# lightbulb128/troy-nova

Hardware: AMD Instinct MI355X
Metric: homomorphic mul+relinearize ops/sec (CKKS mul+relin+rescale), N=16384 (higher is better)
Workload: dtype u64; 1 GPU; CKKS N=16384, 6x50-bit coeff modulus (K=6, L=5): multiply + relinearize + rescale_to_next (BASELINE configs[2]); batch_per_gpu=1024, entry=troyn_ckks_multiply_relinearize_rescale, parallelism=batch-sharded x1, keys broadcast once (RCCL), ranks=1, slowest_rank=0

## Files before the change

### troy-nova_amd/csrc/ntt_kernels.hpp

```cpp
#pragma once
#include "dev_math.hpp"
#include "dev_math_f64.hpp"
#include <type_traits>

namespace troyn {

constexpr int KS_MAX_KEYS = 64;
struct KeyPtrs { const u64* p[KS_MAX_KEYS]; };

struct NttArgs {
    const u64* in;
    u64* out;
    const DevModulus* mods;
    const void* tw;
    long long in_bstride, in_pstride, in_cstride;
    long long out_bstride, out_pstride, out_cstride;
    unsigned pcount, ncomp;
    unsigned table_start, table_count, mode, decomp;
    unsigned reduce_input;
    unsigned stream_loads;
    unsigned load_mode, store_mode;
    unsigned aux_mod;
    unsigned skip_diag;
    unsigned flags;
// ... 258 lines not shown
        const unsigned x0 = (unsigned)x, x1 = (unsigned)(x >> 32), w0 = (unsigned)wq, w1 = (unsigned)(wq >> 32);
        const u64 qh = (u64)x1 * w1 + __umulhi(x1, w0) + __umulhi(x0, w1);
        return w * x + qh * neg_q;
    }
    static __device__ __forceinline__ u64 csub4(u64 v, const Mod& m) {
        const u64 t = v + m.neg_four_q;
        return (long long)t < 0 ? v : t;
    }
    static __device__ __forceinline__ elem mac_zero() { return 0; }
    static __device__ __forceinline__ elem mac_in(u64 canonical, const Mod&) { return canonical; }
    static __device__ __forceinline__ u64 mac_to_lds(elem x, const Mod& m) { return final_fwd(x, m); }
    static __device__ __forceinline__ void mac(elem& acc, elem v, u64 key, const Mod& m) {
        acc = add_mod(acc, barrett128(v * key, mul_hi(v, key), m.q, m.ratio_lo, m.ratio_hi), m.q);
    }
    static __device__ __forceinline__ void mac_fix(elem&, const Mod&) {}
    static __device__ __forceinline__ u64 mac_final(elem acc, const Mod& m) { return final_fwd(acc, m); }
    static constexpr bool HAS_MAC_SHOUP = true;
    static __device__ __forceinline__ void mac_shoup(elem& acc, elem v, u64 key, u64 kq, const Mod& m) {
        acc = csub4(acc + shoup_lazy3(v, key, kq, m.neg_q), m);
    }
    static __device__ __forceinline__ tw_t tw_from_mem(const tw_mem v, const Mod&) { return make_ulonglong2(v.x, v.y); }
    static __device__ __forceinline__ elem load_first(u64 raw, bool reduce, const Mod& m) { return reduce ? barrett64(raw, m.q, m.ratio_hi) : raw; }
    template <int LM> static __device__ __forceinline__ elem load_io(const NttIo& io, u64 raw, bool reduce, const Mod& m) {
        return load_first(ntt_io_load<LM>(io, raw), reduce, m);
    }
    template <int SM> static __device__ __forceinline__ u64 store_prep(elem x, const Mod& m) { return final_fwd(x, m); }
    template <int SM> static __device__ __forceinline__ u64 store_io(const NttIo& io, u64 word, u64 prod, u64 addend, u64 destv, const Mod&) {
        return ntt_io_store<SM>(io, word, prod, addend, destv);
    }
    static __device__ __forceinline__ elem load_mid(u64 raw, const Mod&) { return raw; }
    static __device__ __forceinline__ u64 store_mid(elem x, const Mod&) { return x; }
    static __device__ __forceinline__ elem from_lds(u64 raw) { return raw; }
    static __device__ __forceinline__ u64 to_lds(elem x, const Mod&) { return x; }
    static __device__ __forceinline__ elem mid_fix(elem x, const Mod&) { return x; }
    static __device__ __forceinline__ elem mid_sum(elem x, elem y, const Mod& m) { return csub4(x + y, m); }
    static __device__ __forceinline__ void fwd(elem& a, elem& b, const tw_t w, const Mod& m) {
        const u64 u = csub4(a, m);
        const u64 v = shoup_lazy3(b, w.x, w.y, m.neg_q);
        a = u + v;
        b = u + m.four_q - v;
    }
    static __device__ __forceinline__ void inv(elem& a, elem& b, const tw_t w, const Mod& m) {
        const u64 u = a, v = b;
        a = csub4(u + v, m);
        b = shoup_lazy3(u + m.four_q - v, w.x, w.y, m.neg_q);
    }
    static __device__ __forceinline__ u64 final_inv(elem v, const Mod& m) {
        return shoup_lazy(final_fwd(v, m), m.ninv_op, m.ninv_quo, m.q);
    }
    static __device__ __forceinline__ void inv_fold(elem&, elem&, const Mod&) {}
    static __device__ __forceinline__ elem held_t(elem x, bool, const Mod&) { return x; }
    static __device__ __forceinline__ elem keep(elem x, const Mod& m) { return final_fwd(x, m); }
    static __device__ __forceinline__ elem prod(elem x, elem y, const Mod& m) {
        u64 lo, hi;
        mul128(x, y, lo, hi);
        return barrett128(lo, hi, m.q, m.ratio_lo, m.ratio_hi);
    }
    static __device__ __forceinline__ elem sum(elem x, elem y, const Mod& m) { return add_mod(x, y, m.q); }
    static __device__ __forceinline__ elem inv_in(elem x, const Mod&) { return x; }
    static __device__ __forceinline__ elem prod_in(u64 x, u64 y, const Mod& m) { return prod(x, y, m); }
    static __device__ __forceinline__ elem from_canon(u64 x) { return x; }
    static __device__ __forceinline__ u64 t_residue(u64 raw, bool is_u64, bool aux_bigger, const Mod& m) {
        const u64 t = is_u64 ? raw : f64_to_u64(f64_bits_to_double(raw));
        return aux_bigger ? barrett64(t, m.q, m.ratio_hi) : t;
    }
    template <bool TW> static __device__ __forceinline__ elem tail_in(const NttIo& io, u64 raw_s, u64 raw_l, const Mod& m) {
        const u64 rs = sub_mod(t_residue(raw_s, io.ts_u64, io.aux_bigger, m), io.hm_u, m.q);
        const u64 fl = sub_mod(t_residue(raw_l, io.tl_u64, io.aux2_bigger, m), io.hm2_u, m.q);
        return add_mod(shoup_mul(rs, io.inv.x, io.inv.y, m.q), fl, m.q);
    }
    static __device__ __forceinline__ u64 tail_out(const NttIo& io, u64 prod_word, elem y, const Mod& m) {
        return shoup_mul(sub_mod(prod_word, final_fwd(y, m), m.q), io.inv2.x, io.inv2.y, m.q);
    }
    template <bool TW> static __device__ __forceinline__ u64 last_out(const NttIo& io, elem xr, bool, u64 raw_s, const Mod& m) {
        const u64 ys = final_inv(xr, m);
        const u64 rs = sub_mod(t_residue(raw_s, io.ts_u64, io.aux_bigger, m), io.hm_u, m.q);
        const u64 l = sub_mod(ys, shoup_mul(rs, io.inv.x, io.inv.y, m.q), m.q);
        return add_mod(l, m.q >> 1, m.q);
    }
};

struct ArithF64 {
    static constexpr bool HAS_MAC_SHOUP = false;
    using elem = double;
// ... 37 lines not shown
        }
    }
    template <int SM> static __device__ __forceinline__ u64 store_prep(elem x, const Mod& m) {
        if constexpr (SM == NTT_STORE_PLAIN) return final_fwd(x, m);
        else return f64_double_to_bits(f64_corr(x, m.m));
    }
    template <int SM> static __device__ __forceinline__ u64 store_io(const NttIo& io, u64 word, u64 prod, u64 addend, u64 destv, const Mod& m) {
        if constexpr (SM == NTT_STORE_PLAIN) return word;
        else {
            const double y = f64_bits_to_double(word);
            double d = f64_mulc(f64_from_u64(prod) - y, io.inv_d, io.inv_pd, m.m.p);
            if constexpr (SM == NTT_STORE_KS_FINISH) {
                if (io.add_inplace) d += f64_from_u64(destv);
                if (io.ext1) d += f64_from_u64(addend);
            }
            return f64_canon(d, m.m);
        }
    }
    static __device__ __forceinline__ elem prod_in(u64 x, u64 y, const Mod& m) {
        return f64_mulq(f64_from_u64(x), f64_from_u64(y), m.m.inv_p, m.m.p);
    }
    static __device__ __forceinline__ elem tensor_term(unsigned k, u64 a0, u64 a1, u64 b0, u64 b1, const Mod& m) {
        return k == 0 ? prod_in(a0, b0, m) : prod_in(a0, b1, m) + prod_in(a1, b0, m);
    }
    static __device__ __forceinline__ elem round_fix(u64 x, double aux_q, double aux_half, double hm, const Mod& m) {
        double t = f64_from_u64(x) + aux_half;
        t = (t >= aux_q) ? t - aux_q : t;
        return f64_corr(t - hm, m.m);
    }
    static __device__ __forceinline__ double round_half(double x_canon, const Mod& m) {
        const double t = x_canon + 0.5 * (m.m.p - 1.0);
        return t >= m.m.p ? t - m.m.p : t;
    }
    static __device__ __forceinline__ double held_t(elem x, bool scaled, const Mod& m) {
        const double c = f64_corr(scaled ? x : f64_mulc(x, m.ninv, m.ninv_p, m.m.p), m.m);
        return round_half(c < 0.0 ? c + m.m.p : c, m);
    }
    static __device__ __forceinline__ elem round_fix_t(u64 t_bits, double hm, const Mod& m) { return f64_corr(f64_bits_to_double(t_bits) - hm, m.m); }
    static __device__ __forceinline__ elem round_fix_tw(u64 raw, bool is_u64, double hm, const Mod& m) {
        double t;
        if (is_u64) {
            const double h = (double)(unsigned)(raw >> 30) * 1073741824.0;
            const double lo = (double)((unsigned)raw & 0x3fffffffu);
            t = __builtin_fma(-__builtin_rint(h * m.m.inv_p), m.m.p, h) + lo;
        } else t = f64_bits_to_double(raw);
        return f64_corr(t - hm, m.m);
    }
    static __device__ __forceinline__ elem from_canon(u64 x) { return f64_from_u64(x); }
    template <bool TW> static __device__ __forceinline__ elem tail_in(const NttIo& io, u64 raw_s, u64 raw_l, const Mod& m) {
        const elem rs = TW ? round_fix_tw(raw_s, io.ts_u64, io.hm_d, m) : round_fix_t(raw_s, io.hm_d, m);
        const elem fl = TW ? round_fix_tw(raw_l, io.tl_u64, io.hm2_d, m) : round_fix_t(raw_l, io.hm2_d, m);
        return scale_by(rs, io.inv_d, m) + fl;
    }
    static __device__ __forceinline__ u64 tail_out(const NttIo& io, u64 prod_word, elem y, const Mod& m) {
        return canon_small(scale_by(f64_corr(f64_from_u64(prod_word) - y, m.m), io.inv2_d, m), m);
    }
    template <bool TW> static __device__ __forceinline__ u64 last_out(const NttIo& io, elem xr, bool scaled, u64 raw_s, const Mod& m) {
        const elem ys = scaled ? xr : f64_mulc(xr, m.ninv, m.ninv_p, m.m.p);
        const elem rs = TW ? round_fix_tw(raw_s, io.ts_u64, io.hm_d, m) : round_fix_t(raw_s, io.hm_d, m);
        double lc = f64_corr(ys - scale_by(rs, io.inv_d, m), m.m);
        lc = lc < 0.0 ? lc + m.m.p : lc;
        return f64_double_to_bits(round_half(lc, m));
    }
    static __device__ __forceinline__ u64 canon_small(elem x, const Mod& m) { return f64_to_u64(x < 0.0 ? x + m.m.p : x); }
    static __device__ __forceinline__ elem scale_by(elem x, double inv_d, const Mod& m) { return f64_mulq(x, inv_d, m.m.inv_p, m.m.p); }
    static __device__ __forceinline__ elem load_mid(u64 raw, const Mod& m) { return f64_corr(f64_bits_to_double(raw), m.m); }
    static __device__ __forceinline__ u64 store_mid(elem x, const Mod&) { return f64_double_to_bits(x); }
    static __device__ __forceinline__ elem from_lds(u64 raw) { return f64_bits_to_double(raw); }
    static __device__ __forceinline__ u64 to_lds(elem x, const Mod& m) { return f64_double_to_bits(f64_corr(x, m.m)); }
    static __device__ __forceinline__ elem mid_fix(elem x, const Mod& m) { return f64_corr(x, m.m); }
    static __device__ __forceinline__ elem mid_sum(elem x, elem y, const Mod& m) { return f64_corr(x, m.m) + y; }
    static __device__ __forceinline__ void fwd(elem& a, elem& b, const tw_t w, const Mod& m) {
        const double r = f64_mulq(b, w.x, m.m.inv_p, m.m.p);
        const double u = a;
        a = u + r;
        b = u - r;
    }
    static __device__ __forceinline__ void inv(elem& a, elem& b, const tw_t w, const Mod& m) {
        const double u = a, v = b;
        a = u + v;
        b = f64_mulq(u - v, w.x, m.m.inv_p, m.m.p);
    }
    static __device__ __forceinline__ u64 final_fwd(elem v, const Mod& m) { return f64_canon(v, m.m); }
    static __device__ __forceinline__ u64 final_inv(elem v, const Mod& m) { return f64_canon(f64_mulc(v, m.ninv, m.ninv_p, m.m.p), m.m); }
    static __device__ __forceinline__ elem keep(elem x, const Mod& m) { return f64_corr(x, m.m); }
    static __device__ __forceinline__ elem prod(elem x, elem y, const Mod& m) { return f64_mulq(x, y, m.m.inv_p, m.m.p); }
    static __device__ __forceinline__ elem sum(elem x, elem y, const Mod&) { return x + y; }
    static __device__ __forceinline__ elem inv_in(elem x, const Mod& m) { return f64_corr(x, m.m); }
};

__host__ __device__ constexpr unsigned ntt_wave_bits(int S, int EB, int TB) {
    unsigned m = 0;
    for (int p = 6; p < TB - EB; ++p) m |= 1u << (p < S ? p : p + EB);
    return m;
}

__host__ __device__ constexpr bool ROUNDS_OK(int G, int EB) { return (G + EB - 1) / EB > 1; }

template <class A, int LOGN, int LO, int G, int TB, int EB, bool INV, bool FIRST, bool LAST, bool KSMAC, int IOM, int REGIO = 0, bool HALF = false, bool SHFL = false>
__device__ __forceinline__ void ntt_pass_body(const NttArgs& a, const KeyPtrs* keys, u64* lds, unsigned bid, unsigned t, typename A::elem* xio = nullptr) {
    constexpr int C = TB - G;
    static_assert(!HALF || (!KSMAC && REGIO == 0), "half-word LDS tiles: plain and fused transform kernels only");
    static_assert(REGIO == 0 || REGIO == 3 || REGIO == 4 || (!KSMAC && IOM == 0 && C == 0 && (G + EB - 1) / EB > 1 && (REGIO == 1 ? (!INV && LAST) : (INV && FIRST && (REGIO == 2 || !LAST)))), "register hand-over: last forward / first inverse pass on whole tiles");
    static_assert(REGIO < 3 || REGIO == 5 || (std::is_same<A, ArithF64>::value && !KSMAC && !HALF && C == 0 && LO == 0 && G == TB && TB == LOGN && (G + EB - 1) / EB > 1 &&
                                (REGIO == 3 ? (INV && (IOM == 0 || IOM == NTT_FUSED_LAST_LIMB)) : (REGIO == 4 && !INV && IOM == NTT_FUSED_TAIL_RESCALE))),
                  "held T rows: whole-limb FP64 transforms of the merged chain tail");
    constexpr int E = 1 << EB;
    constexpr unsigned N = 1u << LOGN;
    constexpr int TILE_BITS = LOGN - TB;
    constexpr int NLB = LOGN - LO - G - C;
    static_assert(G >= 1 && C >= 0 && NLB >= 0 && TB >= EB, "bad NTT pass shape");
    constexpr int ROUNDS = (G + EB - 1) / EB;
    static_assert(!KSMAC || (!INV && FIRST && LAST && C == 0 && LO == 0 && ROUNDS > 1), "KSMAC needs a whole-limb forward tile");
    using elem = typename A::elem;
    using tw_t = typename A::tw_t;

    unsigned tile, j, k, b;
    if constexpr (KSMAC) {
        tile = 0; j = 0;
        const unsigned R = a.xcd_groups;
        if (R > 1) {
            const unsigned per = 8u * R, phase = a.batch * R;
            const unsigned q = bid % phase, r = q % per;
            k = (bid / phase) * R + r / 8u;
            b = (q / per) * 8u + (r % 8u);
        } else {
            b = bid % a.batch; k = bid / a.batch;
        }
        if (a.ks_row_mask) k = nth_set_bit(a.ks_row_mask, k);
    } else {
        tile = bid & ((1u << TILE_BITS) - 1); bid >>= TILE_BITS;
        unsigned g;
        if (IOM != 0 && TILE_BITS == 0 && a.xcd_groups) {
            const unsigned per = 8u * a.ncomp, full = (a.xcd_groups / 8u) * per;
            if (bid < full) { const unsigned r = bid % per; j = r / 8u; g = (bid / per) * 8u + (r % 8u); }
            else { const unsigned r = bid - full; j = r % a.ncomp; g = (a.xcd_groups / 8u) * 8u + r / a.ncomp; }
        } else {
            j = bid % a.ncomp; g = bid / a.ncomp;
        }
        k = g % a.pcount;
        b = g / a.pcount;
    }
    const unsigned top = tile >> NLB;
    const unsigned lb = tile & ((1u << NLB) - 1);

    if (!KSMAC && a.skip_diag && k == j && k < a.decomp) return;
    const unsigned mi = KSMAC ? a.table_start + ((k == a.decomp) ? a.table_count - 1 : k) : ntt_table_index(a, k, j);
    const typename A::Mod md = A::make(a.mods[mi]);
    typedef typename A::tw_mem tw_mem;
    typedef const tw_mem __attribute__((address_space(4)))* ctw_ptr;
    unsigned long long tw_addr = (unsigned long long)(reinterpret_cast<const tw_mem*>(a.tw) + (size_t)mi * N);
    ctw_ptr twc = (ctw_ptr)tw_addr;
    auto tw_load = [&](unsigned idx) -> tw_t { const tw_mem v = twc[idx]; return A::tw_from_mem(v, md); };
    const u64* __restrict__ gin = a.in + (long long)b * a.in_bstride + (KSMAC ? 0ll : (long long)k * a.in_pstride + (long long)j * a.in_cstride);
    u64* __restrict__ gout = a.out + (long long)b * a.out_bstride + (KSMAC ? (long long)k * a.out_cstride : (long long)k * a.out_pstride + (long long)j * a.out_cstride);

    auto gindex = [&](unsigned loc) -> unsigned {
        return (top << (LOGN - LO)) | ((loc >> C) << (LOGN - LO - G)) | (lb << C) | (loc & ((1u << C) - 1));
    };
    auto gpart = [](unsigned loc) constexpr -> unsigned { return ((loc >> C) << (LOGN - LO - G)) | (loc & ((1u << C) - 1)); };
    constexpr int LM = (FIRST && !KSMAC && !INV) ? (IOM == 1 ? (int)NTT_LOAD_KS_ROUND : IOM == 2 ? (int)NTT_LOAD_RESCALE : IOM == NTT_IOM_CENTRALIZE ? (int)NTT_LOAD_CENTRALIZE : (int)NTT_LOAD_PLAIN) : (int)NTT_LOAD_PLAIN;
    constexpr int SM = (LAST && !KSMAC && !INV) ? (IOM == 1 ? (int)NTT_STORE_KS_FINISH : IOM == 2 ? (int)NTT_STORE_RESCALE : (int)NTT_STORE_PLAIN) : (int)NTT_STORE_PLAIN;
    constexpr bool FUSED = IOM >= 3 && IOM <= 7;
    constexpr bool F_MULPAIR = IOM == NTT_FUSED_MULPAIR && FIRST;
    constexpr bool F_LAST = IOM == NTT_FUSED_LAST_LIMB || IOM == NTT_FUSED_LAST_LIMB_W, F_TR = IOM == NTT_FUSED_TAIL_RESCALE || IOM == NTT_FUSED_TAIL_RESCALE_W;
    constexpr bool TW = IOM == NTT_FUSED_LAST_LIMB_W || IOM == NTT_FUSED_TAIL_RESCALE_W;
    constexpr bool F_LAST_LD = F_LAST && FIRST, F_LAST_ST = F_LAST && LAST;
    constexpr bool F_TR_LD = F_TR && FIRST, F_TR_ST = F_TR && LAST;
    constexpr bool F_KC_ST = INV && LAST && IOM == 1 && !KSMAC;
    static_assert(!FUSED || !KSMAC, "fused chain: transform kernels");
    static_assert(!TW || std::is_same<A, ArithF64>::value, "the _W variants exist for the FP64 policy (the integer forms read either kind of T row)");
    static_assert(!FUSED || (INV == (IOM == NTT_FUSED_MULPAIR || F_LAST)), "fused chain: transform direction");
    NttIo io;
    if constexpr (FUSED) { io.load_mode = NTT_LOAD_PLAIN; io.store_mode = NTT_STORE_PLAIN; ntt_io_fused(io, a, b, k, j, mi); }
    else if constexpr (LM != NTT_LOAD_PLAIN || SM != NTT_STORE_PLAIN) io = ntt_io_make(a, b, k, j, mi, gout);
    else if constexpr (F_KC_ST) { io = ntt_io_make(a, b, k, j, mi, gout); io.in2 = a.in2 + (long long)b * a.in2_bstride + (long long)k * a.in2_pstride; }
    else { io.load_mode = NTT_LOAD_PLAIN; io.store_mode = NTT_STORE_PLAIN; }
    const long long mul_off = FUSED ? (long long)(a.mul_limb0 + j) * N : 0ll;

    elem x[E];
    elem acc0[KSMAC ? E : 1], acc1[KSMAC ? E : 1];
    const u64* __restrict__ key0 = nullptr;
    const u64* __restrict__ kq0 = nullptr;
    if constexpr (KSMAC) {
        static_for<0, E>([&](auto Rc) { acc0[decltype(Rc)::value] = A::mac_zero(); acc1[decltype(Rc)::value] = A::mac_zero(); });
    }
    const u64* const gin0 = gin;
    auto one_digit = [&](unsigned it) {
    if constexpr (KSMAC) {
        asm volatile("" : "+v"(t));
        unsigned tw_lo = (unsigned)__builtin_amdgcn_readfirstlane((int)(unsigned)tw_addr);
        unsigned tw_hi = (unsigned)__builtin_amdgcn_readfirstlane((int)(unsigned)(tw_addr >> 32));
        asm volatile("" : "+s"(tw_lo), "+s"(tw_hi));
        twc = (ctw_ptr)(((unsigned long long)tw_hi << 32) | tw_lo);
        gin = gin0 + (long long)it * a.in_cstride;
        key0 = keys->p[it] + (size_t)(mi - a.table_start) * N;
        kq0 = a.key_quo ? a.key_quo + (long long)it * a.key_quo_jstride + (size_t)(mi - a.table_start) * N : nullptr;
        if (a.skip_diag && it == k) {
            const unsigned lane = t & 63u, wbase = (t >> 6) * (64u * E);
            const u64* dg = a.ext0 + (long long)b * a.ext0_bstride + (long long)k * a.ext0_cstride;
            static_for<0, E / 2>([&](auto mc) {
// ... 32 lines not shown
            sync();
            static_for<0, E>([&](auto ic) { lds32[wa(ic)] = (unsigned)(w[decltype(ic)::value] >> 32); });
            sync();
            static_for<0, E>([&](auto ic) { constexpr int i = decltype(ic)::value; w[i] = ((u64)lds32[ra(ic)] << 32) | (unsigned)w[i]; });
        }
    };
    auto nothing = [] {};
    auto wave_sync = [] { __builtin_amdgcn_wave_barrier(); };
    auto wg_sync = [] { __syncthreads(); };
    (void)wg_sync;
    static_for<0, ROUNDS>([&](auto rc) {
        constexpr int r = decltype(rc)::value;
        constexpr int BHI = INV ? ((C + (r + 1) * EB - 1 < TB - 1) ? C + (r + 1) * EB - 1 : TB - 1) : TB - 1 - r * EB;
        constexpr int BLO = INV ? C + r * EB : ((TB - (r + 1) * EB > C) ? TB - (r + 1) * EB : C);
        constexpr int S = INV ? ((BLO < TB - EB) ? BLO : TB - EB) : ((TB - (r + 1) * EB > 0) ? TB - (r + 1) * EB : 0);
        static_assert(S >= 0 && S + EB <= TB && BLO >= S && BHI < S + EB && BLO <= BHI, "bad round window");
        const unsigned tlow = t & ((1u << S) - 1);
        const unsigned locbase = tlow | ((t >> S) << (S + EB));
        const unsigned pbase = lds_phys(locbase);
        const unsigned twbase = (S >= 6) ? ((unsigned)__builtin_amdgcn_readfirstlane((int)(t >> S)) << (S + EB)) : locbase;

        constexpr int S_PREV = (r == 0) ? S : (INV ? ((C + (r - 1) * EB < TB - EB) ? C + (r - 1) * EB : TB - EB)
                                                   : ((TB - r * EB > 0) ? TB - r * EB : 0));
        constexpr int S_NEXT = (r == ROUNDS - 1) ? S : (INV ? ((C + (r + 1) * EB < TB - EB) ? C + (r + 1) * EB : TB - EB)
                                                            : ((TB - (r + 2) * EB > 0) ? TB - (r + 2) * EB : 0));
        constexpr bool PRIVATE_IN = (r > 0) && ntt_wave_bits(S_PREV, EB, TB) == ntt_wave_bits(S, EB, TB);
        constexpr bool PRIVATE_OUT = (r < ROUNDS - 1) && ntt_wave_bits(S, EB, TB) == ntt_wave_bits(S_NEXT, EB, TB);
        (void)PRIVATE_IN;

        if constexpr ((REGIO == 2 || REGIO == 5) && r == 0) {
            static_assert(r != 0 || (REGIO != 2 && REGIO != 5) || S == 0, "register hand-over: E consecutive coefficients per thread");
            static_for<0, E>([&](auto Rc) { x[decltype(Rc)::value] = xio[decltype(Rc)::value]; });
        } else if constexpr (REGIO == 4 && r == 0) {
            static_assert(r != 0 || REGIO != 4 || S == TB - EB, "held T rows: the first forward round keeps the words the last inverse round left");
            static_for<0, E>([&](auto Rc) {
                constexpr int R = decltype(Rc)::value;
                x[R] = A::template tail_in<false>(io, f64_double_to_bits(xio[R]), f64_double_to_bits(xio[E + R]), md);
            });
        } else if constexpr (r == 0 && INV && S == 0 && C == 0 && ROUNDS > 1) {
            const unsigned lane = t & 63u, wbase = (t >> 6) * (64u * E);
            const unsigned pown = lds_phys(wbase + lane * E), pidx = lds_phys(wbase + lane * 2u);
            const unsigned gbase = gindex(wbase);
            u64 wv[E];
            static_for<0, E / 2>([&](auto mc) {
                constexpr int m = decltype(mc)::value;
                const unsigned idx = m * 128u + lane * 2u;
                if constexpr (F_MULPAIR) {
                    const ulonglong2 va = ld2_at(io.a1 + mul_off + gbase + m * 128u, lane * 16u, true), vb = ld2_at(io.b1 + mul_off + gbase + m * 128u, lane * 16u, true);
                    wv[2 * m] = A::to_lds(A::prod_in(va.x, vb.x, md), md);
                    wv[2 * m + 1] = A::to_lds(A::prod_in(va.y, vb.y, md), md);
                } else if constexpr (F_LAST_LD) {
                    const ulonglong2 vp = nt_load2(gin + gbase + idx);
                    wv[2 * m] = A::to_lds(A::from_canon(vp.x), md);
                    wv[2 * m + 1] = A::to_lds(A::from_canon(vp.y), md);
                } else {
                    const ulonglong2 v = ld2_at(gin + gbase + m * 128u, lane * 16u, a.stream_loads != 0);
                    wv[2 * m] = ntt_io_load<LM>(io, v.x);
                    wv[2 * m + 1] = ntt_io_load<LM>(io, v.y);
                }
            });
            xchg([&](auto ic) { constexpr int i = decltype(ic)::value; return pidx + lds_off((i / 2) * 128u) + (i & 1); },
                 [&](auto ic) { return pown + (unsigned)decltype(ic)::value; }, wv, wave_sync, nothing);
            static_for<0, E>([&](auto Rc) {
                constexpr int R = decltype(Rc)::value;
                const u64 raw = wv[R];
                if constexpr (F_MULPAIR || F_LAST_LD) x[R] = A::from_lds(raw);
                else if constexpr (FIRST) x[R] = A::load_first(raw, a.reduce_input != 0, md);
                else x[R] = A::load_mid(raw, md);
            });
        } else if constexpr (r == 0) {
            const unsigned lb0 = gindex(locbase) * 8u;
            static_for<0, E>([&](auto Rc) {
                constexpr int R = decltype(Rc)::value;
                constexpr unsigned GR = gpart((unsigned)R << S);
                u64 raw;
                if constexpr (KSMAC) raw = a.stream_loads ? nt_load(gin + gindex(locbase | ((unsigned)R << S))) : gin[gindex(locbase | ((unsigned)R << S))];
                else if constexpr (LM == NTT_LOAD_CENTRALIZE) raw = ((lb0 >> 3) + GR < io.cz_count) ? ld_at(gin + GR, lb0) : 0ull;
                else raw = a.stream_loads ? nt_ld_at(gin + GR, lb0) : ld_at(gin + GR, lb0);
                if constexpr (KSMAC) x[R] = A::load_first(raw, true, md);
                else if constexpr (F_TR_LD) {
                    const u64 raw2 = ld_at(io.in2 + GR, lb0);
                    x[R] = A::template tail_in<TW>(io, raw, raw2, md);
                }
// ... 51 lines not shown
        static_for<0, NLAYERS>([&](auto lc) {
            constexpr int li = decltype(lc)::value;
            constexpr int bit = INV ? BLO + li : BHI - li;
            constexpr int rb = bit - S;
            constexpr int kk = TB - 1 - bit;
            constexpr int l = LO + kk;
            if constexpr (KSMAC || (HALF && !INV)) __builtin_amdgcn_sched_barrier(0);
            if constexpr (HALF && INV && r == 0 && std::is_same<A, ArithF64>::value && (decltype(lc)::value == 1 || decltype(lc)::value == 2)) {
                const unsigned lo = (unsigned)f64_double_to_bits(x[0]);
                asm volatile("v_and_b32 %0, 0, %1" : "=v"(tw_dep) : "v"(lo));
            }
            static_for<0, (E >> (rb + 1))>([&](auto hc) {
                constexpr int hi = decltype(hc)::value;
                const unsigned loc0 = twbase | ((unsigned)(hi << (rb + 1)) << S);
                const unsigned grp = (top << kk) + (loc0 >> (bit + 1));
                const tw_t w = tw_load((INV ? N - (2u << l) + 1 + grp : (1u << l) + grp) + tw_dep);
                static_for<0, (1 << rb)>([&](auto oc) {
                    constexpr int R0 = (hi << (rb + 1)) | decltype(oc)::value;
                    constexpr int R1 = R0 | (1 << rb);
                    if constexpr (!INV) A::fwd(x[R0], x[R1], w, md);
                    else {
                        if constexpr (A::FOLD_NINV && LAST && l == 0) { A::inv_fold(x[R0], x[R1], md); (void)w; }
                        else A::inv(x[R0], x[R1], w, md);
                        if constexpr (A::MID_FIX && NLAYERS == 4 && li == 1) x[R0] = A::mid_fix(x[R0], md);
                    }
                });
            });
        });

        if constexpr (REGIO == 1 && r == ROUNDS - 1) {
            static_assert(r != ROUNDS - 1 || REGIO != 1 || S == 0, "register hand-over: E consecutive coefficients per thread");
            static_for<0, E>([&](auto Rc) { xio[decltype(Rc)::value] = A::keep(x[decltype(Rc)::value], md); });
        } else if constexpr (REGIO == 3 && r == ROUNDS - 1) {
            static_assert(r != ROUNDS - 1 || REGIO != 3 || S == TB - EB, "held T rows: the last inverse round leaves the words the first forward round keeps");
            static_for<0, E>([&](auto Rc) {
                constexpr int R = decltype(Rc)::value;
                constexpr bool scaled = A::FOLD_NINV && ((R >> (EB - 1)) & 1);
                if constexpr (F_LAST_ST) xio[E + R] = f64_bits_to_double(A::template last_out<false>(io, x[R], scaled, f64_double_to_bits(xio[R]), md));
                else xio[R] = A::held_t(x[R], scaled, md);
            });
        } else if constexpr (KSMAC && r == ROUNDS - 1) {
            const unsigned lane = t & 63u, wbase = (t >> 6) * (64u * E);
            const unsigned pown = lds_phys(wbase + lane * E), pidx = lds_phys(wbase + lane * 2u);
            const u64* kp0 = key0 + wbase + lane * 2u;
            const u64* kp1 = kp0 + a.key_pstride;
            ulonglong2 kc0 = *reinterpret_cast<const ulonglong2*>(kp0), kc1 = *reinterpret_cast<const ulonglong2*>(kp1);
            const bool shoup = A::HAS_MAC_SHOUP && kq0 != nullptr;
            const u64* qp0 = shoup ? kq0 + wbase + lane * 2u : kp0;
            const u64* qp1 = qp0 + a.key_pstride;
            ulonglong2 qc0 = make_ulonglong2(0, 0), qc1 = make_ulonglong2(0, 0);
            if constexpr (A::HAS_MAC_SHOUP) { if (shoup) { qc0 = *reinterpret_cast<const ulonglong2*>(qp0); qc1 = *reinterpret_cast<const ulonglong2*>(qp1); } }
            static_for<0, E>([&](auto Rc) {
                constexpr int R = decltype(Rc)::value;
                lds[pown + R] = A::mac_to_lds(x[R], md);
            });
            __builtin_amdgcn_wave_barrier();
            static_for<0, E / 2>([&](auto mc) {
                constexpr int m = decltype(mc)::value;
                ulonglong2 kn0 = kc0, kn1 = kc1, qn0 = qc0, qn1 = qc1;
                if constexpr (m + 1 < E / 2) {
                    kn0 = *reinterpret_cast<const ulonglong2*>(kp0 + (m + 1) * 128u);
                    kn1 = *reinterpret_cast<const ulonglong2*>(kp1 + (m + 1) * 128u);
                    if constexpr (A::HAS_MAC_SHOUP) { if (shoup) {
                        qn0 = *reinterpret_cast<const ulonglong2*>(qp0 + (m + 1) * 128u);
                        qn1 = *reinterpret_cast<const ulonglong2*>(qp1 + (m + 1) * 128u);
                    } }
                }
                const elem v0 = A::from_lds(lds[pidx + lds_off(m * 128u)]), v1 = A::from_lds(lds[pidx + lds_off(m * 128u) + 1]);
                bool done = false;
                if constexpr (A::HAS_MAC_SHOUP) { if (shoup) {
                    A::mac_shoup(acc0[2 * m], v0, kc0.x, qc0.x, md); A::mac_shoup(acc0[2 * m + 1], v1, kc0.y, qc0.y, md);
                    A::mac_shoup(acc1[2 * m], v0, kc1.x, qc1.x, md); A::mac_shoup(acc1[2 * m + 1], v1, kc1.y, qc1.y, md);
                    done = true;
                } }
                if (!done) {
                    A::mac(acc0[2 * m], v0, kc0.x, md); A::mac(acc0[2 * m + 1], v1, kc0.y, md);
                    A::mac(acc1[2 * m], v0, kc1.x, md); A::mac(acc1[2 * m + 1], v1, kc1.y, md);
                }
                kc0 = kn0; kc1 = kn1; qc0 = qn0; qc1 = qn1;
                __builtin_amdgcn_sched_barrier(0);
            });
            __syncthreads();
        } else if constexpr (r == ROUNDS - 1 && !INV && LAST && S == 0 && C == 0 && ROUNDS > 1) {
            const unsigned lane = t & 63u, wbase = (t >> 6) * (64u * E);
            const unsigned pown = lds_phys(wbase + lane * E), pidx = lds_phys(wbase + lane * 2u);
            u64 wv[E];
            static_for<0, E>([&](auto Rc) {
                constexpr int R = decltype(Rc)::value;
                if constexpr (F_TR_ST) wv[R] = A::to_lds(x[R], md);
                else wv[R] = A::template store_prep<SM>(x[R], md);
            });
            const unsigned gbase = gindex(wbase);
            ulonglong2 e0[SM != NTT_STORE_PLAIN ? E / 2 : 1], e1[SM == NTT_STORE_KS_FINISH ? E / 2 : 1], ed[SM == NTT_STORE_KS_FINISH ? E / 2 : 1];
            auto request_operands = [&] {
                if constexpr (SM != NTT_STORE_PLAIN && !HALF) {
                    static_for<0, E / 2>([&](auto mc) {
                        constexpr int m = decltype(mc)::value;
                        e0[m] = *reinterpret_cast<const ulonglong2*>(io.ext0 + gbase + m * 128u + lane * 2u);
                    });
                    if constexpr (SM == NTT_STORE_KS_FINISH) {
                        static_for<0, E / 2>([&](auto mc) { e1[decltype(mc)::value] = make_ulonglong2(0, 0); ed[decltype(mc)::value] = make_ulonglong2(0, 0); });
                        if (io.ext1) static_for<0, E / 2>([&](auto mc) {
                            constexpr int m = decltype(mc)::value;
                            e1[m] = *reinterpret_cast<const ulonglong2*>(io.ext1 + gbase + m * 128u + lane * 2u);
                        });
                        if (io.add_inplace) static_for<0, E / 2>([&](auto mc) {
                            constexpr int m = decltype(mc)::value;
                            ed[m] = *reinterpret_cast<const ulonglong2*>(io.dest + gbase + m * 128u + lane * 2u);
                        });
                    }
                }
            };
            xchg([&](auto ic) { return pown + (unsigned)decltype(ic)::value; },
                 [&](auto ic) { constexpr int i = decltype(ic)::value; return pidx + lds_off((i / 2) * 128u) + (i & 1); }, wv, wave_sync, request_operands);
            static_for<0, E / 2>([&](auto mc) {
                constexpr int m = decltype(mc)::value;
                const unsigned idx = m * 128u + lane * 2u;
                u64 v0 = wv[2 * m], v1 = wv[2 * m + 1];
                if constexpr (F_TR_ST) {
                    const unsigned boff = (gbase + idx) * 8u;
                    ulonglong2 pr;
                    if constexpr (QW > 0) {
                        pr = pq[m];
                        if constexpr (m + QW < E / 2) request_q(std::integral_constant<int, m + QW>{});
                    } else pr = ld2_at(io.ext0, boff, true);
                    v0 = A::tail_out(io, pr.x, A::from_lds(v0), md);
                    v1 = A::tail_out(io, pr.y, A::from_lds(v1), md);
                }
                if constexpr (SM != NTT_STORE_PLAIN && HALF) {
                    const unsigned boff = (gbase + idx) * 8u;
                    const ulonglong2 z = make_ulonglong2(0, 0);
                    const ulonglong2 o0 = ld2_at(io.ext0, boff);
                    ulonglong2 o1 = z, od = z;
                    if constexpr (SM == NTT_STORE_KS_FINISH) {
                        if (io.ext1) o1 = ld2_at(io.ext1, boff);
                        if (io.add_inplace) od = ld2_at(io.dest, boff);
                    }
                    v0 = A::template store_io<SM>(io, v0, o0.x, o1.x, od.x, md);
                    v1 = A::template store_io<SM>(io, v1, o0.y, o1.y, od.y, md);
                } else if constexpr (SM != NTT_STORE_PLAIN) {
                    constexpr int mk = (SM == NTT_STORE_KS_FINISH) ? m : 0;
                    v0 = A::template store_io<SM>(io, v0, e0[m].x, e1[mk].x, ed[mk].x, md);
                    v1 = A::template store_io<SM>(io, v1, e0[m].y, e1[mk].y, ed[mk].y, md);
                }
                nt_store2(gout + gbase + idx, v0, v1);
            });
        } else if constexpr (r == ROUNDS - 1) {
            const unsigned gi0 = gindex(locbase), gb0 = gi0 * 8u;
            static_for<0, E>([&](auto Rc) {
                constexpr int R = decltype(Rc)::value;
                u64 v;
                constexpr unsigned GR = gpart((unsigned)R << S);
                const unsigned gi = gi0 + GR;
                if constexpr (F_LAST_ST) {
                    constexpr bool scaled = A::FOLD_NINV && ((R >> (EB - 1)) & 1);
                    v = A::template last_out<TW>(io, x[R], scaled, io.in2[gi], md);
                } else if constexpr (F_KC_ST) {
                    u64 pw;
                    if constexpr (A::FOLD_NINV && ((R >> (EB - 1)) & 1)) pw = A::final_fwd(x[R], md);
                    else pw = A::final_inv(x[R], md);
                    const elem fixv = A::template load_io<NTT_LOAD_KS_ROUND>(io, io.in2[gi], false, md);
                    v = A::template store_io<NTT_STORE_KS_FINISH>(io, A::store_mid(fixv, md), pw, io.ext1 ? io.ext1[gi] : 0, io.add_inplace ? io.dest[gi] : 0, md);
                } else if constexpr (LAST) {
                    if constexpr (INV && A::FOLD_NINV && ((R >> (EB - 1)) & 1)) v = A::final_fwd(x[R], md);
                    else if constexpr (INV) v = A::final_inv(x[R], md);
                    else if constexpr (SM == NTT_STORE_PLAIN) v = A::final_fwd(x[R], md);
                    else v = A::template store_io<SM>(io, A::template store_prep<SM>(x[R], md), io.ext0[gi],
                                                      (SM == NTT_STORE_KS_FINISH && io.ext1) ? io.ext1[gi] : 0,
                                                      (SM == NTT_STORE_KS_FINISH && io.add_inplace) ? io.dest[gi] : 0, md);
                    if constexpr (INV && IOM == 0 && std::is_same<A, ArithF64>::value) {
                        if (a.flags & NTT_FLAG_STORE_ROUND_HALF) v = f64_double_to_bits(ArithF64::round_half(f64_from_u64(v), md));
                    }
                    if constexpr (INV && IOM == 0 && std::is_same<A, ArithU64>::value) {
                        if (a.flags & NTT_FLAG_STORE_ROUND_HALF) v = add_mod(v, md.q >> 1, md.q);
                    }
                    if constexpr (INV && IOM == NTT_FUSED_MULPAIR && std::is_same<A, ArithF64>::value) {
                        if (a.flags & NTT_FLAG_STORE_F64) v = f64_double_to_bits(f64_from_u64(v));
                    }
                } else {
                    if constexpr (REGIO == 5) { if (a.flags & NTT_FLAG_MID_CARRY) x[R] = A::mid_sum(x[R], A::load_mid(ld_at(gout + GR, gb0), md), md); }
                    v = A::store_mid(x[R], md);
                }
                nt_store_at(gout + GR, gb0, v);
            });
        }
        (void)PRIVATE_OUT;
    });
    };
    if constexpr (KSMAC) {
        for (unsigned it = 0; it < a.decomp; ++it) {
            one_digit(it);
            if ((it & 7u) == 7u) static_for<0, E>([&](auto Rc) { A::mac_fix(acc0[decltype(Rc)::value], md); A::mac_fix(acc1[decltype(Rc)::value], md); });
        }
    }
    else one_digit(0u);
    if constexpr (KSMAC) {
        const unsigned lane = t & 63u, wbase = (t >> 6) * (64u * E);
        static_for<0, E / 2>([&](auto mc) {
            constexpr int m = decltype(mc)::value;
            const unsigned idx = wbase + m * 128u + lane * 2u;
            nt_store2(gout + idx, A::mac_final(acc0[2 * m], md), A::mac_final(acc0[2 * m + 1], md));
            nt_store2(gout + a.out_pstride + idx, A::mac_final(acc1[2 * m], md), A::mac_final(acc1[2 * m + 1], md));
        });
    }
}

template <class A, int LOGN, int LO, int G, int TB, int EB, bool INV, bool FIRST, bool LAST, int IOM, bool HALF = false>
__global__ __launch_bounds__(1 << (TB - EB), HALF ? (2 << (TB - EB - 8)) : 1) void ntt_pass_kernel(NttArgs a) {
    __shared__ u64 lds[(G + EB - 1) / EB > 1 ? (HALF ? (ntt_lds_words(TB) + 1) / 2 : ntt_lds_words(TB)) : 1];
// ... 181 lines not shown
```

### troy-nova_amd/csrc/troyn.hip

```cpp
#include <hip/hip_runtime.h>

#include <algorithm>
#include <atomic>
#include <cstdio>
#include <cstdlib>
#include <cstring>
#include <functional>
#include <memory>
#include <mutex>
#include <string>
#include <vector>

#include "../../include/troyn.h"
#include "behz_kernels.hpp"
#include "behz2_kernels.hpp"
#include "launch.hpp"
#include "crypto_kernels.hpp"
#include "bgv_kernels.hpp"
#include "ring2k_kernels.hpp"
#include "host_math.hpp"
#include "ntt_kernels.hpp"
#include "ksmac_kernels.hpp"
#include "ksmaci_kernels.hpp"
#include "poly_kernels.hpp"
// ... 1565 lines not shown
    x.in_pstride = (long long)(L + 1) * n; x.in_bstride = 2ll * (L + 1) * n;
    x.in2 = c.ws + c.w.spec_intt; x.in2_bstride = 2ll * n; x.in2_pstride = n;
    x.aux_mod = K - 1; x.inv_table = p->d_inv_last + (size_t)K * K + (L - 1);
    x.fused_mode = (!c.last_wide && c.special_wide) ? NTT_FUSED_LAST_LIMB_W : NTT_FUSED_LAST_LIMB;
    x.flags = c.t_flags();
    return x;
}
static NttArgs mrr_tail_args(const MrrCall& c, unsigned j0, unsigned j1) {
    const troyn_plan* p = c.p; const unsigned L = c.L, K = p->K, n = p->n;
    NttArgs x = contiguous_args(p, c.ws + c.w.spec_intt, c.out + (size_t)j0 * n, 2, j1 - j0, j0, j1 - j0, TROYN_IDX_COMPONENTWISE, 0);
    x.in_bstride = 2ll * n; x.in_pstride = n; x.in_cstride = 0;
    x.out_bstride = 2ll * (L - 1) * n; x.out_pstride = (long long)(L - 1) * n;
    x.in2 = c.ws + c.w.last_intt; x.in2_bstride = 2ll * n; x.in2_pstride = n;
    x.aux_mod = K - 1; x.inv_table = p->d_inv_last + (size_t)K * K + j0;
    x.aux2_mod = L - 1; x.inv_table2 = p->d_inv_last + (size_t)L * K + j0;
    x.ext0 = c.poly_prod() + (size_t)j0 * n; x.ext0_bstride = 2ll * (L + 1) * n; x.ext0_pstride = (long long)(L + 1) * n; x.ext0_cstride = n;
    x.fused_mode = (class_by_policy(p, j0) && c.t_flags()) ? NTT_FUSED_TAIL_RESCALE_W : NTT_FUSED_TAIL_RESCALE;
    x.flags = c.t_flags();
    return x;
}

static int mrr_tail_merged(const MrrCall& c, bool quartet) {
    const troyn_plan* p = c.p; const unsigned L = c.L, K = p->K, n = p->n;
    const LaunchCtx lc = launch_ctx(p, c.s);
    if (quartet) {
        u64* rows = c.poly_prod() + (size_t)(L - 1) * n;
        NttArgs pa = contiguous_args(p, rows, rows, 2, 2, L - 1, K - (L - 1), TROYN_IDX_KS_SKIP_FINALS, 1);
        pa.in_pstride = pa.out_pstride = (long long)(L + 1) * n; pa.in_bstride = pa.out_bstride = 2ll * (L + 1) * n;
        prep_direct(p, pa, true, true);
        launch_small_pass(p->log_n, true, 0, pa, c.batch * 4, lc);
        LAUNCH_CHECK();
    }
    NttArgs sp = special_rows_args(p, c.poly_prod(), nullptr, L);
    if (!quartet) sp.flags = NTT_FLAG_STORE_ROUND_HALF;
    prep_direct(p, sp, true, true);
    NttArgs la = mrr_last_args(c);
    prep_direct(p, la, true, true);
    NttArgs ta = mrr_tail_args(c, 0, L - 1);
    prep_direct(p, ta, true, false);
    if (!quartet) {
        launch_mrr_tail(p->log_n, c.batch, sp, la, ta, c.s);
        LAUNCH_CHECK();
        return TROYN_OK;
    }
    launch_mrr_quartet(p->log_n, c.batch, sp, la, ta, c.s, !p->opt.mrr_small_serial && is_small_launch(c.batch * 2 * (size_t)(L - 1)));
    LAUNCH_CHECK();
    as_input_of(ta, ta);
    ta.reduce_input = 0;
    launch_small_pass(p->log_n, true, 1, ta, c.batch * 2 * (L - 1), lc);
    LAUNCH_CHECK();
    return TROYN_OK;
}

static int mrr_chain(const troyn_plan* p, uint32_t L, const KsRows& rows, const u64* a, const u64* b, const double* kf, const ulonglong2* ki, u64* out, u64* ws,
                     const MrrLayout& w, size_t batch, hipStream_t s, const KeyPtrs* raw = nullptr) {
    const MrrCall c{p, L, a, b, out, ws, w, batch, s, mrr_all_f64(p, L), !class_by_policy(p, p->K - 1), !class_by_policy(p, L - 1)};
    int rc;
    if ((rc = mrr_digits(c))) return rc;
    if ((rc = mrr_inner_product(c, rows, kf, ki, raw))) return rc;
    if (c.all_f64 && (small_tail_wanted(p, batch * 2 * (size_t)(L - 1)) || (p->log_n == 15 && !p->opt.mrr_small_off))) return mrr_tail_merged(c, true);
    if (c.all_f64 && p->log_n == 14 && !p->opt.mrr_small_off) return mrr_tail_merged(c, false);
    {
        NttArgs x = special_rows_args(p, c.poly_prod(), ws + w.spec_intt, L);
        x.flags = NTT_FLAG_STORE_ROUND_HALF;
        if ((rc = launch_ntt(p, x, batch, true, s))) return rc;
    }
    if ((rc = launch_ntt(p, mrr_last_args(c), batch, true, s))) return rc;
// ... 1317 lines not shown
```

Baseline: 300,900 ops/s.

## Keep FP64 held rows centred and skip redundant corrections in lean N=16384 transforms

For whole-limb FP64 transforms at logN 14 (mul-pair and tail-rescale fused chains), LDS stores skip the modular correction, and held rows between the inverse and forward passes are kept as centred residues instead of round-half canonical values. The tail input then avoids re-applying the half-modulus offset. Digit outputs of the mul-pair inverse are written directly as FP64 bits or as a 2^52-offset integer encoding, with no separate canonical step. The special-rows kernel no longer sets the store-round-half flag in the non-quartet path. This trims arithmetic from the NTT store and load paths, but it relies on lazy FP64 ranges staying within precision bounds and on the centred convention being consistent across kernels.

```diff
diff --git a/troy-nova_amd/csrc/ntt_kernels.hpp b/troy-nova_amd/csrc/ntt_kernels.hpp
--- a/troy-nova_amd/csrc/ntt_kernels.hpp
+++ b/troy-nova_amd/csrc/ntt_kernels.hpp
@@ -314,6 +314,7 @@
     static __device__ __forceinline__ u64 store_mid(elem x, const Mod&) { return x; }
     static __device__ __forceinline__ elem from_lds(u64 raw) { return raw; }
     static __device__ __forceinline__ u64 to_lds(elem x, const Mod&) { return x; }
+    static __device__ __forceinline__ u64 to_lds_raw(elem x, const Mod&) { return x; }
     static __device__ __forceinline__ elem mid_fix(elem x, const Mod&) { return x; }
     static __device__ __forceinline__ elem mid_sum(elem x, elem y, const Mod& m) { return csub4(x + y, m); }
     static __device__ __forceinline__ void fwd(elem& a, elem& b, const tw_t w, const Mod& m) {
@@ -331,7 +332,10 @@
         return shoup_lazy(final_fwd(v, m), m.ninv_op, m.ninv_quo, m.q);
     }
     static __device__ __forceinline__ void inv_fold(elem&, elem&, const Mod&) {}
-    static __device__ __forceinline__ elem held_t(elem x, bool, const Mod&) { return x; }
+    static __device__ __forceinline__ elem held_c(elem x, bool, const Mod&) { return x; }
+    static __device__ __forceinline__ elem held_last(const NttIo&, elem x, bool, elem, const Mod&) { return x; }
+    static __device__ __forceinline__ elem held_tail_in(const NttIo&, elem x, elem, const Mod&) { return x; }
+    static __device__ __forceinline__ u64 digit_word(elem x, bool, double, unsigned, const Mod&) { return x; }
     static __device__ __forceinline__ elem keep(elem x, const Mod& m) { return final_fwd(x, m); }
     static __device__ __forceinline__ elem prod(elem x, elem y, const Mod& m) {
         u64 lo, hi;
@@ -435,9 +439,25 @@
         const double t = x_canon + 0.5 * (m.m.p - 1.0);
         return t >= m.m.p ? t - m.m.p : t;
     }
-    static __device__ __forceinline__ double held_t(elem x, bool scaled, const Mod& m) {
-        const double c = f64_corr(scaled ? x : f64_mulc(x, m.ninv, m.ninv_p, m.m.p), m.m);
-        return round_half(c < 0.0 ? c + m.m.p : c, m);
+    static __device__ __forceinline__ double centred(double x, const Mod& m) {
+        const double c = f64_corr(x, m.m);
+        const double step = __builtin_fabs(c) > 0.5 * (m.m.p - 1.0) ? __builtin_copysign(m.m.p, c) : 0.0;
+        return c - step;
+    }
+    static __device__ __forceinline__ double held_c(elem x, bool scaled, const Mod& m) {
+        return centred(scaled ? x : f64_mulc(x, m.ninv, m.ninv_p, m.m.p), m);
+    }
+    static __device__ __forceinline__ double held_last(const NttIo& io, elem xr, bool scaled, double cs, const Mod& m) {
+        const elem ys = scaled ? xr : f64_mulc(xr, m.ninv, m.ninv_p, m.m.p);
+        return centred(ys - scale_by(cs, io.inv_d, m), m);
+    }
+    static __device__ __forceinline__ elem held_tail_in(const NttIo& io, double cs, double cl, const Mod& m) {
+        return scale_by(cs, io.inv_d, m) + cl;
+    }
+    static __device__ __forceinline__ u64 digit_word(elem x, bool scaled, double add, unsigned mask_hi, const Mod& m) {
+        double c = f64_corr(scaled ? x : f64_mulc(x, m.ninv, m.ninv_p, m.m.p), m.m);
+        c = c < 0.0 ? c + m.m.p : c;
+        return f64_double_to_bits(c + add) & (((u64)mask_hi << 32) | 0xffffffffull);
     }
     static __device__ __forceinline__ elem round_fix_t(u64 t_bits, double hm, const Mod& m) { return f64_corr(f64_bits_to_double(t_bits) - hm, m.m); }
     static __device__ __forceinline__ elem round_fix_tw(u64 raw, bool is_u64, double hm, const Mod& m) {
@@ -471,6 +491,7 @@
     static __device__ __forceinline__ u64 store_mid(elem x, const Mod&) { return f64_double_to_bits(x); }
     static __device__ __forceinline__ elem from_lds(u64 raw) { return f64_bits_to_double(raw); }
     static __device__ __forceinline__ u64 to_lds(elem x, const Mod& m) { return f64_double_to_bits(f64_corr(x, m.m)); }
+    static __device__ __forceinline__ u64 to_lds_raw(elem x, const Mod&) { return f64_double_to_bits(x); }
     static __device__ __forceinline__ elem mid_fix(elem x, const Mod& m) { return f64_corr(x, m.m); }
     static __device__ __forceinline__ elem mid_sum(elem x, elem y, const Mod& m) { return f64_corr(x, m.m) + y; }
     static __device__ __forceinline__ void fwd(elem& a, elem& b, const tw_t w, const Mod& m) {
@@ -507,7 +528,7 @@
     static_assert(REGIO == 0 || REGIO == 3 || REGIO == 4 || (!KSMAC && IOM == 0 && C == 0 && (G + EB - 1) / EB > 1 && (REGIO == 1 ? (!INV && LAST) : (INV && FIRST && (REGIO == 2 || !LAST)))), "register hand-over: last forward / first inverse pass on whole tiles");
     static_assert(REGIO < 3 || REGIO == 5 || (std::is_same<A, ArithF64>::value && !KSMAC && !HALF && C == 0 && LO == 0 && G == TB && TB == LOGN && (G + EB - 1) / EB > 1 &&
                                 (REGIO == 3 ? (INV && (IOM == 0 || IOM == NTT_FUSED_LAST_LIMB)) : (REGIO == 4 && !INV && IOM == NTT_FUSED_TAIL_RESCALE))),
-                  "held T rows: whole-limb FP64 transforms of the merged chain tail");
+                  "held rows: whole-limb FP64 transforms of the merged chain tail");
     constexpr int E = 1 << EB;
     constexpr unsigned N = 1u << LOGN;
     constexpr int TILE_BITS = LOGN - TB;
@@ -570,6 +591,7 @@
     constexpr bool TW = IOM == NTT_FUSED_LAST_LIMB_W || IOM == NTT_FUSED_TAIL_RESCALE_W;
     constexpr bool F_LAST_LD = F_LAST && FIRST, F_LAST_ST = F_LAST && LAST;
     constexpr bool F_TR_LD = F_TR && FIRST, F_TR_ST = F_TR && LAST;
+    constexpr bool LEAN = std::is_same<A, ArithF64>::value && LOGN == 14 && !HALF && FIRST && LAST && C == 0 && (IOM == NTT_FUSED_MULPAIR || IOM == NTT_FUSED_TAIL_RESCALE);
     constexpr bool F_KC_ST = INV && LAST && IOM == 1 && !KSMAC;
     static_assert(!FUSED || !KSMAC, "fused chain: transform kernels");
     static_assert(!TW || std::is_same<A, ArithF64>::value, "the _W variants exist for the FP64 policy (the integer forms read either kind of T row)");
@@ -668,10 +690,10 @@
             static_assert(r != 0 || (REGIO != 2 && REGIO != 5) || S == 0, "register hand-over: E consecutive coefficients per thread");
             static_for<0, E>([&](auto Rc) { x[decltype(Rc)::value] = xio[decltype(Rc)::value]; });
         } else if constexpr (REGIO == 4 && r == 0) {
-            static_assert(r != 0 || REGIO != 4 || S == TB - EB, "held T rows: the first forward round keeps the words the last inverse round left");
+            static_assert(r != 0 || REGIO != 4 || S == TB - EB, "held rows: the first forward round keeps the words the last inverse round left");
             static_for<0, E>([&](auto Rc) {
                 constexpr int R = decltype(Rc)::value;
-                x[R] = A::template tail_in<false>(io, f64_double_to_bits(xio[R]), f64_double_to_bits(xio[E + R]), md);
+                x[R] = A::held_tail_in(io, xio[R], xio[E + R], md);
             });
         } else if constexpr (r == 0 && INV && S == 0 && C == 0 && ROUNDS > 1) {
             const unsigned lane = t & 63u, wbase = (t >> 6) * (64u * E);
@@ -683,8 +705,13 @@
                 const unsigned idx = m * 128u + lane * 2u;
                 if constexpr (F_MULPAIR) {
                     const ulonglong2 va = ld2_at(io.a1 + mul_off + gbase + m * 128u, lane * 16u, true), vb = ld2_at(io.b1 + mul_off + gbase + m * 128u, lane * 16u, true);
-                    wv[2 * m] = A::to_lds(A::prod_in(va.x, vb.x, md), md);
-                    wv[2 * m + 1] = A::to_lds(A::prod_in(va.y, vb.y, md), md);
+                    if constexpr (LEAN) {
+                        wv[2 * m] = A::to_lds_raw(A::prod_in(va.x, vb.x, md), md);
+                        wv[2 * m + 1] = A::to_lds_raw(A::prod_in(va.y, vb.y, md), md);
+                    } else {
+                        wv[2 * m] = A::to_lds(A::prod_in(va.x, vb.x, md), md);
+                        wv[2 * m + 1] = A::to_lds(A::prod_in(va.y, vb.y, md), md);
+                    }
                 } else if constexpr (F_LAST_LD) {
                     const ulonglong2 vp = nt_load2(gin + gbase + idx);
                     wv[2 * m] = A::to_lds(A::from_canon(vp.x), md);
@@ -802,12 +829,12 @@
             static_assert(r != ROUNDS - 1 || REGIO != 1 || S == 0, "register hand-over: E consecutive coefficients per thread");
             static_for<0, E>([&](auto Rc) { xio[decltype(Rc)::value] = A::keep(x[decltype(Rc)::value], md); });
         } else if constexpr (REGIO == 3 && r == ROUNDS - 1) {
-            static_assert(r != ROUNDS - 1 || REGIO != 3 || S == TB - EB, "held T rows: the last inverse round leaves the words the first forward round keeps");
+            static_assert(r != ROUNDS - 1 || REGIO != 3 || S == TB - EB, "held rows: the last inverse round leaves the words the first forward round keeps");
             static_for<0, E>([&](auto Rc) {
                 constexpr int R = decltype(Rc)::value;
                 constexpr bool scaled = A::FOLD_NINV && ((R >> (EB - 1)) & 1);
-                if constexpr (F_LAST_ST) xio[E + R] = f64_bits_to_double(A::template last_out<false>(io, x[R], scaled, f64_double_to_bits(xio[R]), md));
-                else xio[R] = A::held_t(x[R], scaled, md);
+                if constexpr (F_LAST_ST) xio[E + R] = A::held_last(io, x[R], scaled, xio[R], md);
+                else xio[R] = A::held_c(x[R], scaled, md);
             });
         } else if constexpr (KSMAC && r == ROUNDS - 1) {
             const unsigned lane = t & 63u, wbase = (t >> 6) * (64u * E);
@@ -857,7 +884,8 @@
             u64 wv[E];
             static_for<0, E>([&](auto Rc) {
                 constexpr int R = decltype(Rc)::value;
-                if constexpr (F_TR_ST) wv[R] = A::to_lds(x[R], md);
+                if constexpr (F_TR_ST && LEAN) wv[R] = A::to_lds_raw(x[R], md);
+                else if constexpr (F_TR_ST) wv[R] = A::to_lds(x[R], md);
                 else wv[R] = A::template store_prep<SM>(x[R], md);
             });
             const unsigned gbase = gindex(wbase);
@@ -917,12 +945,19 @@
             });
         } else if constexpr (r == ROUNDS - 1) {
             const unsigned gi0 = gindex(locbase), gb0 = gi0 * 8u;
+            constexpr bool LEAN_DIGITS = LEAN && INV && IOM == NTT_FUSED_MULPAIR;
+            const bool digits_f64 = LEAN_DIGITS && (a.flags & NTT_FLAG_STORE_F64) != 0;
+            const double dg_add = digits_f64 ? 0.0 : F64_TWO52;
+            const unsigned dg_mask_hi = digits_f64 ? 0xffffffffu : 0x000fffffu;
+            (void)dg_add; (void)dg_mask_hi;
             static_for<0, E>([&](auto Rc) {
                 constexpr int R = decltype(Rc)::value;
                 u64 v;
                 constexpr unsigned GR = gpart((unsigned)R << S);
                 const unsigned gi = gi0 + GR;
-                if constexpr (F_LAST_ST) {
+                if constexpr (LEAN_DIGITS) {
+                    v = A::digit_word(x[R], A::FOLD_NINV && ((R >> (EB - 1)) & 1), dg_add, dg_mask_hi, md);
+                } else if constexpr (F_LAST_ST) {
                     constexpr bool scaled = A::FOLD_NINV && ((R >> (EB - 1)) & 1);
                     v = A::template last_out<TW>(io, x[R], scaled, io.in2[gi], md);
                 } else if constexpr (F_KC_ST) {
@@ -944,7 +979,7 @@
                     if constexpr (INV && IOM == 0 && std::is_same<A, ArithU64>::value) {
                         if (a.flags & NTT_FLAG_STORE_ROUND_HALF) v = add_mod(v, md.q >> 1, md.q);
                     }
-                    if constexpr (INV && IOM == NTT_FUSED_MULPAIR && std::is_same<A, ArithF64>::value) {
+                    if constexpr (!LEAN && INV && IOM == NTT_FUSED_MULPAIR && std::is_same<A, ArithF64>::value) {
                         if (a.flags & NTT_FLAG_STORE_F64) v = f64_double_to_bits(f64_from_u64(v));
                     }
                 } else {
diff --git a/troy-nova_amd/csrc/troyn.hip b/troy-nova_amd/csrc/troyn.hip
--- a/troy-nova_amd/csrc/troyn.hip
+++ b/troy-nova_amd/csrc/troyn.hip
@@ -1621,7 +1621,6 @@
         LAUNCH_CHECK();
     }
     NttArgs sp = special_rows_args(p, c.poly_prod(), nullptr, L);
-    if (!quartet) sp.flags = NTT_FLAG_STORE_ROUND_HALF;
     prep_direct(p, sp, true, true);
     NttArgs la = mrr_last_args(c);
     prep_direct(p, la, true, true);
```

Result: faster. 308,300 ops/s, median of 6 (+2.5%).
